# martinruenz/maskfusion

Measured on NVIDIA H100. Metric: frames/sec on 640x480 .klg replay, higher is better.
Workload: dtype f32

## Files before the change

### maskfusion_b200/csrc/mf_surfel.cu

```cuda
#include "mf_common.cuh"
#include "mf_kernels.h"
#include "mf_host.h"

namespace mfb {

#define MAX_POINT_SIZE 2047.0f

__global__ void __launch_bounds__(256) k_index_project(const float4* __restrict__ pos, const float4* __restrict__ col,
                                                       const uint32_t* __restrict__ countPtr, const DevPose* __restrict__ dpose, Cam cam, int W, int H,
                                                       float maxDepth, float ftime, float ftimeDelta,
                                                       unsigned long long* __restrict__ key)
{
    const Rt tinv = dpose->tinv;
    const uint32_t count = *countPtr;
    for (uint32_t id = blockIdx.x * blockDim.x + threadIdx.x; id < count; id += gridDim.x * blockDim.x) {
        float4 p = ldStream(pos + id);
        float lastTime = ldStream(col + id).w;
        float3 ph = xform(tinv, make_float3(p.x, p.y, p.z));
        if (ph.z > maxDepth || ph.z <= 0 || ftime - lastTime > ftimeDelta) continue;
        float x = ((cam.fx * ph.x) / ph.z) + cam.cx;
        float y = ((cam.fy * ph.y) / ph.z) + cam.cy;
        float zn = ph.z / maxDepth;
        if (!(zn < 1.0f)) continue;
        float fx_ = floorf(x), fy_ = floorf(y);
// ... 307 lines not shown
        for (uint32_t i = lane; i < staged; i += 32) cand[gbase + i] = sBuf[warp][i];
        __syncwarp();
        staged = 0;
    };
    const uint32_t stride = gridDim.x * blockDim.x;
    float4 vpN = make_float4(0, 0, 0, 0), vcN = vpN;
    { const uint32_t e0 = blockIdx.x * blockDim.x + threadIdx.x; if (e0 < count) { vpN = pos[e0]; vcN = col[e0]; } }
    for (uint32_t base = blockIdx.x * blockDim.x; base < total; base += stride) {
        const uint32_t e = base + threadIdx.x;
        bool valid = false, need = false, noWindow = false;
        const bool isOld = e < count;
        float4 vp = vpN, vc = vcN;
        if (e + stride < count) { vpN = pos[e + stride]; vcN = col[e + stride]; }
        if (isOld) valid = true;
        else if (e < total) { uint32_t p = e - count; if (aflag[p] == 2) { vp = m0[p]; vc = m1[p]; valid = true; } }
        if (valid) {
            float3 lp = xform(P.tinv, make_float3(vp.x, vp.y, vp.z));
            float x = ((P.cam.fx * lp.x) / lp.z) + P.cam.cx;
            float y = ((P.cam.fy * lp.y) / lp.z) + P.cam.cy;
            need = ftime - vc.w < P.ftimeDelta && lp.z > 0 && x > 0 && y > 0 && x < cols && y < rows;
            if (indexKey && isOld && !(lp.z > indexMaxDepth || lp.z <= 0 || ftime - vc.w > P.ftimeDelta)) {
                const float zn = lp.z / indexMaxDepth;
                const float fx_ = floorf(x), fy_ = floorf(y);
                if (zn < 1.0f && fx_ >= 0 && fy_ >= 0 && fx_ < cols && fy_ < rows) {
                    const unsigned long long k = ((unsigned long long)__float_as_uint(zn) << 32) | e;
                    unsigned long long* dst = indexKey + ((int)fy_ * P.W + (int)fx_);
                    if (k < *dst) atomicMin(dst, k);
                    if (!need) { need = true; noWindow = true; }
                }
            }
            if (!need) {
                const float w0 = vp.w, t0 = vc.w;
                bool k = cleanFinish(vp, vc, x, y, lp.z, 0, 0, P, depthFilt, mask);
                if (isOld) { if (vp.w != w0) pos[e].w = vp.w; if (vc.w != t0) col[e].w = vc.w; }
                else { uint32_t p = e - count; m0[p].w = vp.w; m1[p].w = vc.w; }
                keep[e] = k ? 1 : 0;
            }
        } else if (e < total) keep[e] = 0;
        const unsigned nb = __ballot_sync(0xffffffffu, need);
        if (nb) {
            if (staged + 32 > CAND_BUF / 8) flush();
            if (need) sBuf[warp][staged + __popc(nb & ((1u << lane) - 1))] = noWindow ? (e | 0x80000000u) : e;
            staged += (uint32_t)__popc(nb);
            __syncwarp();
        }
    }
    if (staged) flush();
}

template <bool PACKED>
__global__ void __launch_bounds__(256, 4) k_clean_p2(float4* __restrict__ pos, float4* __restrict__ col, const float4* __restrict__ nrm,
                                                  const uint32_t* __restrict__ countPtr, float4* __restrict__ m0, float4* __restrict__ m1,
                                                  const float4* __restrict__ m2, CleanParams P, const DevPose* __restrict__ dpose, CleanTexels cleanTex,
                                                  const float* __restrict__ depthFilt, const uint8_t* __restrict__ mask, uint8_t* __restrict__ keep,
                                                  const uint32_t* __restrict__ cand, const uint32_t* __restrict__ candCount)
{
    P.tinv = dpose->tinv;
    const uint32_t count = *countPtr, n = *candCount;
    const float cols = (float)P.W, rows = (float)P.H;
    for (uint32_t j = blockIdx.x * blockDim.x + threadIdx.x; j < n; j += gridDim.x * blockDim.x) {
        const uint32_t ce_ = cand[j];
        const bool noWindow = (ce_ >> 31) != 0;
        const uint32_t e = ce_ & 0x7fffffffu;
        const bool isOld = e < count;
        const uint32_t p = e - count;
        float4 vp, vc, vn;
        if (isOld) { vp = pos[e]; vc = col[e]; vn = nrm[e]; } else { vp = m0[p]; vc = m1[p]; vn = m2[p]; }
        const float w0 = vp.w, t0 = vc.w;
        float3 lp = xform(P.tinv, make_float3(vp.x, vp.y, vp.z));
        float x = ((P.cam.fx * lp.x) / lp.z) + P.cam.cx;
        float y = ((P.cam.fy * lp.y) / lp.z) + P.cam.cy;
        float3 ln = normalize3(rotate(P.tinv, make_float3(vn.x, vn.y, vn.z)));
        CleanEntry ce; ce.xn = x / cols; ce.yn = y / rows; ce.lx = lp.x; ce.ly = lp.y; ce.lz = lp.z; ce.init = vc.z; ce.rad = vn.w; ce.lnz = fabsf(ln.z);
        int c1 = 0, c2 = 0;
        if (!noWindow) cleanWindow<PACKED>(ce, P, cleanTex, c1, c2);
        bool k = cleanFinish(vp, vc, x, y, lp.z, c1, c2, P, depthFilt, mask);
        if (isOld) { if (vp.w != w0) pos[e].w = vp.w; if (vc.w != t0) col[e].w = vc.w; }
        else { m0[p].w = vp.w; m1[p].w = vc.w; }
        keep[e] = k ? 1 : 0;
    }
}

__global__ void __launch_bounds__(256) k_keep_block_sums(const uint8_t* __restrict__ keep, const uint32_t* __restrict__ countPtr, int Ppix,
                                                         uint32_t* __restrict__ blockSums, uint32_t* __restrict__ candCount, uint32_t* __restrict__ ticket)
{
    const uint32_t total = *countPtr + (uint32_t)Ppix;
    const uint32_t nblk = (total + SCAN_BLOCK - 1) / SCAN_BLOCK;
    if (blockIdx.x == 0 && threadIdx.x == 0) { *candCount = 0; *ticket = 0; }
    const uint32_t lane = threadIdx.x & 31, gw = (blockIdx.x * blockDim.x + threadIdx.x) >> 5, nw = (gridDim.x * blockDim.x) >> 5;
    for (uint32_t blk = gw; blk < nblk; blk += nw) {
        const uint32_t e0 = blk * SCAN_BLOCK + lane * 16;
        uint4 v = make_uint4(0, 0, 0, 0);
        if (e0 < total) v = *reinterpret_cast<const uint4*>(keep + e0);
        if (e0 < total && total - e0 < 16) {
            const uint32_t r = total - e0;
            uint32_t w[4] = {v.x, v.y, v.z, v.w};
#pragma unroll
            for (int q = 0; q < 4; ++q) { const uint32_t lo = (uint32_t)q * 4; w[q] = r <= lo ? 0u : (r - lo >= 4 ? w[q] : (w[q] & ((1u << (8 * (r - lo))) - 1u))); }
            v = make_uint4(w[0], w[1], w[2], w[3]);
        }
        uint32_t c = __popc(v.x & 0x01010101u) + __popc(v.y & 0x01010101u) + __popc(v.z & 0x01010101u) + __popc(v.w & 0x01010101u);
#pragma unroll
        for (int off = 16; off > 0; off >>= 1) c += __shfl_xor_sync(0xffffffffu, c, off);
        if (lane == 0) blockSums[blk] = c;
    }
}

__global__ void __launch_bounds__(1024) k_scan_block_sums(uint32_t* __restrict__ blockSums, const uint32_t* __restrict__ countPtr,
                                                          int extra, uint32_t capacity, uint32_t* __restrict__ newCount, uint32_t* __restrict__ firstMoved)
{
    const uint32_t total = *countPtr + (uint32_t)extra;
    const uint32_t nblk = (total + SCAN_BLOCK - 1) / SCAN_BLOCK;
    __shared__ uint32_t wtot[32];
    __shared__ uint32_t sFirst;
    if (threadIdx.x == 0) sFirst = nblk;
    __syncthreads();
    const uint32_t per = (nblk + 1023) / 1024;
    const uint32_t b0 = threadIdx.x * per, b1 = min(b0 + per, nblk);
    uint32_t run = 0, first = 0xffffffffu;
    for (uint32_t i = b0; i < b1; ++i) { const uint32_t v = blockSums[i]; run += v; if (v != SCAN_BLOCK && first == 0xffffffffu) first = i; }
    if (first != 0xffffffffu) atomicMin(&sFirst, first);
    const int lane = threadIdx.x & 31, warp = threadIdx.x >> 5;
    uint32_t incl = run;
#pragma unroll
    for (int off = 1; off < 32; off <<= 1) { const uint32_t t = __shfl_up_sync(0xffffffffu, incl, off); if (lane >= off) incl += t; }
    if (lane == 31) wtot[warp] = incl;
    __syncthreads();
    if (warp == 0) {
        uint32_t w = wtot[lane], wi = w;
#pragma unroll
        for (int off = 1; off < 32; off <<= 1) { const uint32_t t = __shfl_up_sync(0xffffffffu, wi, off); if (lane >= off) wi += t; }
        wtot[lane] = wi - w;
        if (lane == 31) { *newCount = wi < capacity ? wi : capacity; }
    }
    __syncthreads();
    uint32_t offs = wtot[warp] + incl - run;
    for (uint32_t i = b0; i < b1; ++i) { const uint32_t v = blockSums[i]; blockSums[i] = offs; offs += v; }
    if (threadIdx.x == 0) { firstMoved[0] = sFirst; firstMoved[1] = nblk; }
}

__global__ void __launch_bounds__(SCAN_BLOCK) k_clean_scatter(const float4* __restrict__ pos, const float4* __restrict__ col, const float4* __restrict__ nrm,
                                                              const uint32_t* __restrict__ countPtr, const float4* __restrict__ m0,
                                                              const float4* __restrict__ m1, const float4* __restrict__ m2, int Ppix,
                                                              const uint8_t* __restrict__ keep, const uint32_t* __restrict__ blockOffs,
                                                              uint32_t capacity, float4* __restrict__ opos, float4* __restrict__ ocol,
                                                              float4* __restrict__ onrm)
{
    const uint32_t count = *countPtr;
    const uint32_t total = count + (uint32_t)Ppix;
    const uint32_t nblk = (total + SCAN_BLOCK - 1) / SCAN_BLOCK;
    __shared__ uint32_t wsum[SCAN_BLOCK / 32];
    for (uint32_t blk = blockIdx.x; blk < nblk; blk += gridDim.x) {
        uint32_t e = blk * SCAN_BLOCK + threadIdx.x;
        bool k = e < total && keep[e];
        unsigned bal = __ballot_sync(0xffffffffu, k);
        int lane = threadIdx.x & 31, warp = threadIdx.x >> 5;
        if (lane == 0) wsum[warp] = __popc(bal);
        __syncthreads();
        uint32_t woff = 0;
        for (int w = 0; w < warp; ++w) woff += wsum[w];
        uint32_t dst = blockOffs[blk] + woff + __popc(bal & ((1u << lane) - 1));
        if (k && dst < capacity) {
            float4 a, b, c;
            if (e < count) { a = ldStream(pos + e); b = ldStream(col + e); c = ldStream(nrm + e); }
            else { uint32_t p = e - count; a = m0[p]; b = m1[p]; c = m2[p]; }
            stStream(opos + dst, a); stStream(ocol + dst, b); stStream(onrm + dst, c);
        }
        __syncthreads();
    }
}

__global__ void __launch_bounds__(SCAN_BLOCK) k_clean_compact(float4* __restrict__ pos, float4* __restrict__ col, float4* __restrict__ nrm,
                                                              const uint32_t* __restrict__ countPtr, const float4* __restrict__ m0,
                                                              const float4* __restrict__ m1, const float4* __restrict__ m2, int Ppix,
                                                              const uint8_t* __restrict__ keep, const uint32_t* __restrict__ blockOffs,
                                                              uint32_t capacity, uint32_t* __restrict__ ticket, uint32_t* __restrict__ loaded,
                                                              const uint32_t* __restrict__ firstMoved, uint32_t epoch)
{
    const uint32_t count = *countPtr;
    const uint32_t total = count + (uint32_t)Ppix;
    const uint32_t nblk = (total + SCAN_BLOCK - 1) / SCAN_BLOCK;
    const uint32_t first = *firstMoved;
    __shared__ uint32_t wsum[SCAN_BLOCK / 32];
    __shared__ uint32_t sBlk[2];
    const int lane = threadIdx.x & 31, warp = threadIdx.x >> 5;
    if (threadIdx.x == 0) sBlk[0] = first + atomicAdd(ticket, 1u);
    __syncthreads();
    for (uint32_t it = 0;; ++it) {
        const uint32_t blk = sBlk[it & 1];
        if (blk >= nblk) break;
        if (threadIdx.x == 0) sBlk[(it + 1) & 1] = first + atomicAdd(ticket, 1u);
        const uint32_t e = blk * SCAN_BLOCK + threadIdx.x;
        const bool k = e < total && keep[e];
        const unsigned bal = __ballot_sync(0xffffffffu, k);
        if (lane == 0) wsum[warp] = __popc(bal);
        __syncthreads();
        uint32_t woff = 0, nb = 0;
#pragma unroll
        for (int w = 0; w < SCAN_BLOCK / 32; ++w) { const uint32_t c = wsum[w]; if (w < warp) woff += c; nb += c; }
        const uint32_t off = blockOffs[blk];
        const uint32_t dst = off + woff + __popc(bal & ((1u << lane) - 1));
        const bool isOld = e < count;
        const bool move = k && dst < capacity && !(isOld && dst == e);
        float4 a = make_float4(0, 0, 0, 0), b = a, c = a;
        if (move) {
            if (isOld) { a = __ldcg(pos + e); b = __ldcg(col + e); c = __ldcg(nrm + e); }
            else { const uint32_t p = e - count; a = m0[p]; b = m1[p]; c = m2[p]; }
        }
        const unsigned probe = __float_as_uint(a.x) & __float_as_uint(b.y) & __float_as_uint(c.z);
        __syncthreads_or(probe == 0x7fedcba9u);
        if (threadIdx.x == 0) {
            asm volatile("st.release.gpu.global.u32 [%0], %1;" ::"l"(loaded + blk), "r"(epoch) : "memory");
            if (nb) {
                const uint32_t s0 = off / SCAN_BLOCK, s1 = (off + nb - 1) / SCAN_BLOCK;
                for (uint32_t s = s0; s <= s1 && s < blk; ++s) {
                    if (s < first) continue;
                    unsigned v;
                    do { asm volatile("ld.acquire.gpu.global.u32 %0, [%1];" : "=r"(v) : "l"(loaded + s) : "memory"); } while (v != epoch);
                }
            }
        }
        __syncthreads();
        if (move) { stStream(pos + dst, a); stStream(col + dst, b); stStream(nrm + dst, c); }
    }
}

struct SplatVS { float3 pos; float conf; float3 n; float rad, size, xw, yw; bool ok; };

MF_D SplatVS splatVertex(float4 p, float4 c, float4 nr, const Rt& tinv, Cam cam, int W, int H, float maxDepth,
                         float confThreshold, float ftime, float fmaxTime, float ftimeDelta)
{
    SplatVS o; o.ok = false;
    float3 ph = xform(tinv, make_float3(p.x, p.y, p.z));
    if (ph.z > maxDepth || ph.z < 0 || p.w < confThreshold || ftime - c.w > ftimeDelta || c.w > fmaxTime) return o;
    o.pos = ph; o.conf = p.w;
    o.n = normalize3(rotate(tinv, make_float3(nr.x, nr.y, nr.z)));
    o.rad = nr.w;
    float3 x1 = normalize3(make_float3(o.n.y - o.n.z, -o.n.x, o.n.x));
    x1 = make_float3(x1.x * o.rad * 1.41421356f, x1.y * o.rad * 1.41421356f, x1.z * o.rad * 1.41421356f);
    float3 y1 = cross3(o.n, x1);
    float px[4], py[4];
#pragma unroll
    for (int q = 0; q < 4; ++q) {
        float3 d = (q == 0 || q == 3) ? x1 : y1;
        float sg = (q < 2) ? 1.0f : -1.0f;
        float3 pp = make_float3(ph.x + sg * d.x, ph.y + sg * d.y, ph.z + sg * d.z);
        px[q] = ((cam.fx * pp.x) / pp.z) + cam.cx;
        py[q] = ((cam.fy * pp.y) / pp.z) + cam.cy;
    }
    float xmin = fminf(px[0], fminf(px[1], fminf(px[2], px[3]))), xmax = fmaxf(px[0], fmaxf(px[1], fmaxf(px[2], px[3])));
    float ymin = fminf(py[0], fminf(py[1], fminf(py[2], py[3]))), ymax = fmaxf(py[0], fmaxf(py[1], fmaxf(py[2], py[3])));
    float sz = fmaxf(0.0f, fmaxf(fabsf(xmax - xmin), fabsf(ymax - ymin)));
    if (!(sz >= 1.0f)) sz = 1.0f;
    if (sz > MAX_POINT_SIZE) sz = MAX_POINT_SIZE;
    o.size = sz;
    o.xw = ((cam.fx * ph.x) / ph.z) + cam.cx;
    o.yw = ((cam.fy * ph.y) / ph.z) + cam.cy;
    if (!(o.xw >= 0 && o.xw <= (float)W && o.yw >= 0 && o.yw <= (float)H)) return o;
    if (!(ph.z / maxDepth <= 1.0f)) return o;
    o.ok = true;
    return o;
}

MF_D float3 pixelRay(Cam cam, float fcx, float fcy)
{
    return normalize3(make_float3((fcx - cam.cx) / cam.fx, (fcy - cam.cy) / cam.fy, 1.0f));
}
__global__ void k_ray_table(Cam cam, int W, int H, float4* __restrict__ tab)
{
    int px = blockIdx.x * blockDim.x + threadIdx.x, py = blockIdx.y * blockDim.y + threadIdx.y;
    if (px >= W || py >= H) return;
    float3 l = pixelRay(cam, (float)px + 0.5f, (float)py + 0.5f);
    tab[py * W + px] = make_float4(l.x, l.y, l.z, 0.f);
}

MF_D bool splatFragmentRay(const SplatVS& v, float3 l, float3& cp)
{
    float t = dot3(v.pos, v.n) / dot3(l, v.n);
    cp = make_float3(t * l.x, t * l.y, t * l.z);
    float sqrRad = v.rad * v.rad;
    float3 d = sub3(cp, v.pos);
    return !(dot3(d, d) > sqrRad);
}
MF_D bool splatFragment(const SplatVS& v, Cam cam, float fcx, float fcy, float3& cp) { return splatFragmentRay(v, pixelRay(cam, fcx, fcy), cp); }

MF_D void splatRange(const SplatVS& v, int W, int H, int& x0, int& x1, int& y0, int& y1)
{
    float h = v.size * 0.5f;
    float lo = ceilf(v.xw - h - 0.5f), hi = ceilf(v.xw + h - 0.5f) - 1.0f;
    x0 = lo < 0 ? 0 : (int)lo; x1 = hi > (float)(W - 1) ? W - 1 : (int)hi;
    lo = ceilf(v.yw - h - 0.5f); hi = ceilf(v.yw + h - 0.5f) - 1.0f;
    y0 = lo < 0 ? 0 : (int)lo; y1 = hi > (float)(H - 1) ? H - 1 : (int)hi;
}

#define SPLAT_SEG 8
#ifndef SPLAT_BS
#define SPLAT_BS 128
#endif
#ifndef SPLAT_MIN_BLOCKS
#define SPLAT_MIN_BLOCKS 8
#endif
#define SPLAT_Q 64

struct __align__(16) SplatEntry { float px, py, pz, pn, nx, ny, nz, rad; int x0, y0, w; uint32_t id; };

MF_D void splatExact(const SplatEntry& e, int pix, const float4* __restrict__ rayTab, unsigned long long* __restrict__ key, float maxDepth)
{
    SplatVS sv; sv.pos = make_float3(e.px, e.py, e.pz); sv.n = make_float3(e.nx, e.ny, e.nz); sv.rad = e.rad;
    const float4 l4 = __ldg(rayTab + pix);
    float3 cp;
    if (!splatFragmentRay(sv, make_float3(l4.x, l4.y, l4.z), cp)) return;
    const float fd = (cp.z / (2 * maxDepth)) + 0.5f;
    if (!(fd >= 0.0f && fd < 1.0f)) return;
    const unsigned long long k = ((unsigned long long)__float_as_uint(fd) << 32) | e.id;
    if (k < key[pix]) atomicMin(key + pix, k);
}

__global__ void __launch_bounds__(SPLAT_BS, SPLAT_MIN_BLOCKS) k_splat_project(const float4* __restrict__ pos, const float4* __restrict__ col, const float4* __restrict__ nrm,
                                                       const uint32_t* __restrict__ countPtr, const DevPose* __restrict__ dpose, Cam cam, int W, int H,
                                                       float maxDepth, float confThreshold, float ftime, float fmaxTime, float ftimeDelta,
                                                       uint32_t drawBase, const float4* __restrict__ rayTab, unsigned long long* __restrict__ key)
{
    constexpr int NW = SPLAT_BS / 32;
    static_assert(SPLAT_BS % 32 == 0 && SPLAT_BS <= 256, "the queue packs the entry slot into 8 bits");
    __shared__ SplatEntry ent[2][SPLAT_BS];
    __shared__ int offs[2][SPLAT_BS];
    __shared__ __align__(16) float4 spos[SPLAT_BS];
    __shared__ uint32_t queue[NW][SPLAT_Q];
    __shared__ int wtot[NW], wcnt[NW];
    __shared__ Rt tinv;
    __shared__ float inv2md;
    __shared__ __align__(8) unsigned long long bar;
    const uint32_t count = *countPtr;
    const int lane = threadIdx.x & 31, warp = threadIdx.x >> 5;
    const uint32_t stride = gridDim.x * SPLAT_BS;
    const unsigned barAddr = (unsigned)__cvta_generic_to_shared(&bar);
    const unsigned sposAddr = (unsigned)__cvta_generic_to_shared(spos);
    auto fetch = [&](uint32_t b) {
        const unsigned bytes = min((uint32_t)SPLAT_BS, count - b) * 16u;
        asm volatile("mbarrier.arrive.expect_tx.shared::cta.b64 _, [%0], %1;" ::"r"(barAddr), "r"(bytes) : "memory");
        asm volatile("cp.async.bulk.shared::cluster.global.mbarrier::complete_tx::bytes [%0], [%1], %2, [%3];"
                     ::"r"(sposAddr), "l"(pos + b), "r"(bytes), "r"(barAddr) : "memory");
    };
    if (threadIdx.x < 12) tinv.m[threadIdx.x] = dpose->tinv.m[threadIdx.x];
    if (threadIdx.x == 0) {
        inv2md = 1.0f / (2 * maxDepth);
        asm volatile("mbarrier.init.shared::cta.b64 [%0], 1;" ::"r"(barAddr));
        asm volatile("fence.mbarrier_init.release.cluster;" ::: "memory");
        if (blockIdx.x * SPLAT_BS < count) fetch(blockIdx.x * SPLAT_BS);
    }
    __syncthreads();
    unsigned parity = 0;
    for (uint32_t base = blockIdx.x * SPLAT_BS; base < count; base += stride, parity ^= 1u) {
        const uint32_t id = base + threadIdx.x;
        SplatVS v; v.ok = false;
        int x0 = 0, x1 = -1, y0 = 0, y1 = -1;
        asm volatile(
            "{\n\t.reg .pred p;\n\t"
            "SPLAT_WAIT:\n\t"
            "mbarrier.try_wait.parity.shared::cta.b64 p, [%0], %1;\n\t"
            "@!p bra SPLAT_WAIT;\n\t}" ::"r"(barAddr), "r"(parity) : "memory");
        if (id < count) {
            const float4 p = spos[threadIdx.x];
            float3 ph = xform(tinv, make_float3(p.x, p.y, p.z));
            const float cxw = ((cam.fx * ph.x) / ph.z) + cam.cx, cyw = ((cam.fy * ph.y) / ph.z) + cam.cy;
            if (!(ph.z > maxDepth || ph.z < 0 || p.w < confThreshold) && cxw >= 0 && cxw <= (float)W && cyw >= 0 && cyw <= (float)H) {
                float4 c = ldStream(col + id), nr = ldStream(nrm + id);
                v = splatVertex(p, c, nr, tinv, cam, W, H, maxDepth, confThreshold, ftime, fmaxTime, ftimeDelta);
                if (v.ok) splatRange(v, W, H, x0, x1, y0, y1);
            }
        }
        const bool draw = v.ok && x1 >= x0 && y1 >= y0;
        const int nunit = draw ? (y1 - y0 + 1) * ((x1 - x0 + SPLAT_SEG) / SPLAT_SEG) : 0;
        int incl = nunit;
#pragma unroll
        for (int o = 1; o < 32; o <<= 1) { int t = __shfl_up_sync(0xffffffffu, incl, o); if (lane >= o) incl += t; }
        unsigned db = __ballot_sync(0xffffffffu, draw);
        if (lane == 31) wtot[warp] = incl;
        if (lane == 0) wcnt[warp] = __popc(db);
        __syncthreads();
        if (threadIdx.x == 0 && base + stride < count) {
            asm volatile("fence.proxy.async.shared::cta;" ::: "memory");
            fetch(base + stride);
        }
        SplatEntry* __restrict__ E = ent[parity];
        int* __restrict__ O = offs[parity];
        int fbase = 0, sbase = 0, total = 0, nent = 0;
#pragma unroll
        for (int w = 0; w < NW; ++w) { if (w < warp) { fbase += wtot[w]; sbase += wcnt[w]; } total += wtot[w]; nent += wcnt[w]; }
        if (draw) {
            const int slot = sbase + __popc(db & ((1u << lane) - 1));
            SplatEntry e; e.px = v.pos.x; e.py = v.pos.y; e.pz = v.pos.z; e.pn = dot3(v.pos, v.n); e.nx = v.n.x; e.ny = v.n.y; e.nz = v.n.z; e.rad = v.rad;
            e.x0 = x0; e.y0 = y0; e.w = x1 - x0 + 1; e.id = drawBase + id;
            E[slot] = e;
            O[slot] = fbase + incl - nunit;
        }
        __syncthreads();
        uint32_t* __restrict__ q = queue[warp];
        int qn = 0;
        for (int ub = threadIdx.x - lane + blockIdx.y * SPLAT_BS; ub < total; ub += SPLAT_BS * gridDim.y) {
            const int u = ub + lane;
            int slot = 0, pix = 0, n = 0;
            if (u < total) {
                int lo = 0, hi = nent - 1;
                while (lo < hi) { int mid = (lo + hi + 1) >> 1; if (O[mid] <= u) lo = mid; else hi = mid - 1; }
                slot = lo;
                const int t = u - O[slot], w = E[slot].w, x0e = E[slot].x0;
                const int nseg = (w + SPLAT_SEG - 1) / SPLAT_SEG;
                const int row = t / nseg, xs = x0e + (t - row * nseg) * SPLAT_SEG;
                n = min(SPLAT_SEG, x0e + w - xs);
                pix = (E[slot].y0 + row) * W + xs;
            }
            const int nmax = __reduce_max_sync(0xffffffffu, n);
            for (int i = 0; i < nmax; ++i, ++pix) {
                bool cand = false;
                if (i < n) {
                    const float4 pp = *reinterpret_cast<const float4*>(&E[slot].px), nr = *reinterpret_cast<const float4*>(&E[slot].nx);
                    const float4 l4 = __ldg(rayTab + pix);
                    const unsigned long long cur = key[pix];
                    const float ta = __fdividef(pp.w, dot3(make_float3(l4.x, l4.y, l4.z), make_float3(nr.x, nr.y, nr.z)));
                    cand = cur == KEY_EMPTY || !(__fmaf_rn(ta * l4.z, inv2md, 0.5f) > __uint_as_float((unsigned)(cur >> 32)) * 1.00001f);
                    if (cand) {
                        const float ax = __fmaf_rn(ta, l4.x, -pp.x), ay = __fmaf_rn(ta, l4.y, -pp.y), az = __fmaf_rn(ta, l4.z, -pp.z);
                        const float re = nr.w + 8e-6f * fabsf(ta);
                        cand = !(__fmaf_rn(ax, ax, __fmaf_rn(ay, ay, az * az)) > re * re * 1.0001f);
                    }
                }
                const unsigned m = __ballot_sync(0xffffffffu, cand);
                if (cand) q[qn + __popc(m & ((1u << lane) - 1))] = (uint32_t)pix << 8 | (uint32_t)slot;
                qn += __popc(m);
                if (qn >= 32) {
                    qn -= 32;
                    __syncwarp();
                    const uint32_t it = q[qn + lane];
                    __syncwarp();
                    splatExact(E[it & 255u], (int)(it >> 8), rayTab, key, maxDepth);
                }
            }
        }
        __syncwarp();
        if (lane < qn) {
            const uint32_t it = q[lane];
            splatExact(E[it & 255u], (int)(it >> 8), rayTab, key, maxDepth);
        }
    }
}

__global__ void k_splat_resolve(const float4* __restrict__ pos, const float4* __restrict__ col, const float4* __restrict__ nrm,
                                const DevPose* __restrict__ dpose, Cam cam, int W, int H, float maxDepth, float confThreshold, float ftime, float fmaxTime,
                                float ftimeDelta, const float4* __restrict__ rayTab, unsigned long long* __restrict__ key,
                                uchar4* __restrict__ image, float4* __restrict__ vertexConf, float4* __restrict__ normalRad,
                                uint16_t* __restrict__ timeTex,
                                int doFill, const float* __restrict__ depthFilt, const uchar4* __restrict__ rgb, int ptVN, int ptImg,
                                uchar4* __restrict__ fillImage, float4* __restrict__ fillVertex, float4* __restrict__ fillNormal,
                                uint32_t* __restrict__ nonBlackSamples)
{
    const Rt tinv = dpose->tinv;
    int px = blockIdx.x * blockDim.x + threadIdx.x, py = blockIdx.y * blockDim.y + threadIdx.y;
    if (px >= W || py >= H) return;
    int i = py * W + px;
    unsigned long long k = key[i];
    uchar4 im = make_uchar4(0, 0, 0, 0);
    float4 vc = make_float4(0, 0, 0, 0), nr = vc;
    uint16_t tt = 0;
    if (k != KEY_EMPTY) {
        key[i] = KEY_EMPTY;
        uint32_t id = (uint32_t)(k & 0xffffffffull);
        float4 p = pos[id], c = col[id], n = nrm[id];
        SplatVS v = splatVertex(p, c, n, tinv, cam, W, H, maxDepth, confThreshold, ftime, fmaxTime, ftimeDelta);
        float3 cp; float fcx = (float)px + 0.5f, fcy = (float)py + 0.5f;
        const float4 l4 = __ldg(rayTab + i);
        splatFragmentRay(v, make_float3(l4.x, l4.y, l4.z), cp);
        float3 cl = decodeColor(c.x);
        im = make_uchar4((uint8_t)(int)floorf(cl.x * 255.0f + 0.5f), (uint8_t)(int)floorf(cl.y * 255.0f + 0.5f),
                         (uint8_t)(int)floorf(cl.z * 255.0f + 0.5f), 255);
        float z = cp.z;
        vc = make_float4((fcx - cam.cx) * z * (1.f / cam.fx), (fcy - cam.cy) * z * (1.f / cam.fy), z, v.conf);
        nr = make_float4(v.n.x, v.n.y, v.n.z, v.rad);
        tt = (uint16_t)(uint32_t)c.z;
    }
    image[i] = im; vertexConf[i] = vc; normalRad[i] = nr; timeTex[i] = tt;
    if (nonBlackSamples && (px % 20) == 10 && (py % 20) == 10 && px / 20 < W / 20 && py / 20 < H / 20) {
        if (im.x > 0 && im.y > 0 && im.z > 0) atomicAdd(nonBlackSamples, 1u);
    }
    if (doFill) {
        const float ifx = 1.0f / cam.fx, ify = 1.0f / cam.fy;
        float3 vp = getVertex(depthFilt, W, H, px, py, (float)px, (float)py, cam, ifx, ify);
        fillVertex[i] = (vc.z == 0 || ptVN) ? make_float4(vp.x, vp.y, vp.z, 1.f) : vc;
        if (nr.z == 0 || ptVN) {
            float3 n = normalForward(depthFilt, W, H, px, py, cam, ifx, ify, vp);
            fillNormal[i] = make_float4(n.x, n.y, n.z, 1.f);
        } else fillNormal[i] = nr;
        float sum = ((float)im.x / 255.0f + (float)im.y / 255.0f) + (float)im.z / 255.0f;
        fillImage[i] = (sum == 0 || ptImg) ? rgb[i] : im;
    }
}

__global__ void __launch_bounds__(SCAN_BLOCK) k_init_flags(const float* __restrict__ depthRaw, const float* __restrict__ depthFilt,
                                                           int W, int H, float maxDepth, uint8_t* __restrict__ fr, uint8_t* __restrict__ ff,
                                                           uint32_t* __restrict__ sumR, uint32_t* __restrict__ sumF)
{
    const int P = W * H;
    __shared__ uint32_t ws[2][SCAN_BLOCK / 32];
    int p = blockIdx.x * SCAN_BLOCK + threadIdx.x;
    bool kr = false, kf = false;
    if (p < P) {
        int i = p / H, j = p - i * H;
        float zr = depthRaw[j * W + i], zf = depthFilt[j * W + i];
        kr = !(zr <= 0 || zr > maxDepth);
        kf = !(zf <= 0 || zf > maxDepth);
        fr[p] = kr; ff[p] = kf;
    }
    unsigned br = __ballot_sync(0xffffffffu, kr), bf = __ballot_sync(0xffffffffu, kf);
    if ((threadIdx.x & 31) == 0) { ws[0][threadIdx.x >> 5] = __popc(br); ws[1][threadIdx.x >> 5] = __popc(bf); }
    __syncthreads();
    if (threadIdx.x == 0) {
        uint32_t a = 0, b = 0;
        for (int w = 0; w < SCAN_BLOCK / 32; ++w) { a += ws[0][w]; b += ws[1][w]; }
        sumR[blockIdx.x] = a; sumF[blockIdx.x] = b;
    }
}

__global__ void __launch_bounds__(SCAN_BLOCK) k_init_scatter(const uchar4* __restrict__ rgb, const float* __restrict__ depthRaw,
                                                             const float* __restrict__ depthFilt, Cam cam, int W, int H, int time,
                                                             const uint8_t* __restrict__ fr, const uint8_t* __restrict__ ff,
                                                             const uint32_t* __restrict__ offR, const uint32_t* __restrict__ offF,
                                                             uint32_t capacity, float4* __restrict__ pos, float4* __restrict__ col,
                                                             float4* __restrict__ nrm)
{
    const int P = W * H;
    __shared__ uint32_t ws[2][SCAN_BLOCK / 32];
    int p = blockIdx.x * SCAN_BLOCK + threadIdx.x;
    bool kr = p < P && fr[p], kf = p < P && ff[p];
    unsigned br = __ballot_sync(0xffffffffu, kr), bf = __ballot_sync(0xffffffffu, kf);
    int lane = threadIdx.x & 31, warp = threadIdx.x >> 5;
    if (lane == 0) { ws[0][warp] = __popc(br); ws[1][warp] = __popc(bf); }
    __syncthreads();
    uint32_t wr = 0, wf = 0;
    for (int w = 0; w < warp; ++w) { wr += ws[0][w]; wf += ws[1][w]; }
    if (p >= P) return;
    int i = p / H, j = p - i * H;
    const float ifx = 1.0f / cam.fx, ify = 1.0f / cam.fy;
    float tcx = (float)(((double)((float)i / (float)W)) + 1.0 / (double)(2 * (float)W));
    float tcy = (float)(((double)((float)j / (float)H)) + 1.0 / (double)(2 * (float)H));
    float x = tcx * (float)W, y = tcy * (float)H;
    if (kr) {
        uint32_t dst = offR[blockIdx.x] + wr + __popc(br & ((1u << lane) - 1));
        if (dst < capacity) {
            float3 vp = getVertex(depthRaw, W, H, i, j, x, y, cam, ifx, ify);
            uchar4 c8 = rgb[j * W + i];
            pos[dst] = make_float4(vp.x, vp.y, vp.z, surfelConfidence(x, y, 1.0f, cam.cx, cam.cy));
            col[dst] = make_float4(encodeColor((float)c8.x / 255.0f, (float)c8.y / 255.0f, (float)c8.z / 255.0f), 0.f, 1.f, (float)time);
        }
    }
    if (kf) {
        uint32_t dst = offF[blockIdx.x] + wf + __popc(bf & ((1u << lane) - 1));
        if (dst < capacity) {
            float3 vp = getVertex(depthFilt, W, H, i, j, x, y, cam, ifx, ify);
            float3 nl = normalCentral(depthFilt, W, H, i, j, x, y, cam, ifx, ify, vp);
            nrm[dst] = make_float4(nl.x, nl.y, nl.z, surfelRadius(vp.z, nl.z, ifx, ify));
        }
    }
}

__global__ void __launch_bounds__(1024) k_scan_small(uint32_t* __restrict__ a, int n, uint32_t capacity, uint32_t* __restrict__ total)
{
    __shared__ uint32_t sh[1024];
    __shared__ uint32_t carry;
    if (threadIdx.x == 0) carry = 0;
    __syncthreads();
    for (int base = 0; base < n; base += 1024) {
        int i = base + threadIdx.x;
        uint32_t v = i < n ? a[i] : 0;
        sh[threadIdx.x] = v;
        __syncthreads();
        for (int off = 1; off < 1024; off <<= 1) {
            uint32_t t = threadIdx.x >= off ? sh[threadIdx.x - off] : 0;
            __syncthreads();
            sh[threadIdx.x] += t;
            __syncthreads();
        }
        uint32_t incl = sh[threadIdx.x];
        if (i < n) a[i] = carry + incl - v;
        __syncthreads();
        if (threadIdx.x == 1023) carry += incl;
        __syncthreads();
    }
    if (threadIdx.x == 0 && total) *total = carry < capacity ? carry : capacity;
}

__global__ void k_fill_u32(uint32_t* p, uint32_t v, size_t n)
{
    size_t i = (size_t)blockIdx.x * blockDim.x + threadIdx.x;
    if (i < n) p[i] = v;
}
__global__ void k_fill_u64(unsigned long long* p, unsigned long long v, size_t n)
{
    size_t i = (size_t)blockIdx.x * blockDim.x + threadIdx.x;
    if (i < n) p[i] = v;
}
__global__ void k_zero_f4(float4* p, uint32_t from, uint32_t to)
{
    uint32_t i = from + blockIdx.x * blockDim.x + threadIdx.x;
    if (i < to) p[i] = make_float4(0, 0, 0, 0);
}

__global__ void k_planes_to_aos(const float4* __restrict__ pos, const float4* __restrict__ col, const float4* __restrict__ nrm, uint32_t n, float4* __restrict__ out)
{
    uint32_t i = blockIdx.x * blockDim.x + threadIdx.x;
    if (i >= n) return;
    out[(size_t)i * 3] = pos[i]; out[(size_t)i * 3 + 1] = col[i]; out[(size_t)i * 3 + 2] = nrm[i];
}
__global__ void k_aos_to_planes(const float4* __restrict__ in, uint32_t n, float4* __restrict__ pos, float4* __restrict__ col, float4* __restrict__ nrm)
{
    uint32_t i = blockIdx.x * blockDim.x + threadIdx.x;
    if (i >= n) return;
    pos[i] = in[(size_t)i * 3]; col[i] = in[(size_t)i * 3 + 1]; nrm[i] = in[(size_t)i * 3 + 2];
}

static int g_numSMs = 0;
void set_num_sms(int n) { g_numSMs = n > 0 ? n : 132; }
int num_sms()
{
    if (!g_numSMs) { int dev = 0, n = 0; cudaGetDevice(&dev); cudaDeviceGetAttribute(&n, cudaDevAttrMultiProcessorCount, dev); set_num_sms(n); }
    return g_numSMs;
}
static inline int persistentBlocks(int perSM) { return num_sms() * perSM; }

struct Pose2 { float p[16], l[16]; };
__global__ void k_set_pose(DevPose* d, Pose2 in)
{
    if (threadIdx.x == 0 && blockIdx.x == 0) derivePose(d, in.p, in.l);
}
void launch_set_pose(DevPose* d, const float* pose16, const float* lastPose16, Enq q)
{
    Pose2 in;
    for (int k = 0; k < 16; ++k) { in.p[k] = pose16[k]; in.l[k] = lastPose16[k]; }
    launch(q, nullptr, k_set_pose, 1, 32, 0, d, in);
}

void launch_fill_u32(uint32_t* p, uint32_t v, size_t n, Enq q) { if (n) launch(q, nullptr, k_fill_u32, (unsigned)((n + 255) / 256), 256, 0, p, v, n); }
void launch_fill_u64(uint64_t* p, uint64_t v, size_t n, Enq q) { if (n) launch(q, nullptr, k_fill_u64, (unsigned)((n + 255) / 256), 256, 0, (unsigned long long*)p, v, n); }

void launch_predict_indices(const SurfelPlanes& sp, const uint32_t* count, const DevPose* tinv, Cam cam, int W, int H, float maxDepth, int time,
                            int timeDelta, uint64_t* key, uint32_t* idx, float4* vertConf, float4* colorTime, float4* normRad, float4* cleanTex, float cleanConf, Enq q)
{
    launch(q, "k_index_project", k_index_project, persistentBlocks(8), 256, 0, sp.pos, sp.col, count, tinv, cam, W, H, maxDepth, (float)time, (float)timeDelta,
           (unsigned long long*)key);
    int P = W * H;
    launch(q, "k_index_resolve", k_index_resolve, (P + 255) / 256, 256, 0, sp.pos, sp.col, sp.nrm, tinv, P, (unsigned long long*)key, idx, vertConf, colorTime, normRad, cleanTex, cleanConf, (float)time);
}

void launch_associate(const uchar4* rgb, const float* depthRaw, const float* depthFilt, const uint8_t* mask, const uint32_t* idx,
                      const float4* vertConf, const float4* normRad, const DevPose* pose, Cam cam, int W, int H, float maxDepth, int time,
                      float weighting, uint8_t maskID, uint8_t* flag, uint32_t* best, float4* const* meas, uint32_t* slot, Enq q)
{
    dim3 b(32, 8), g((W + 31) / 32, (H + 7) / 8);
    launch(q, "k_associate", k_associate, g, b, 0, rgb, depthRaw, depthFilt, mask, idx, vertConf, normRad, pose, cam, W, H, maxDepth, time, weighting, maskID,
           flag, best, meas[0], meas[1], meas[2], slot);
}

void launch_fuse_update(const uint8_t* flag, const uint32_t* best, float4* const* meas, uint32_t* slot, int P, int time,
                        const SurfelPlanes& sp, Enq q)
{
    launch(q, "k_fuse_update", k_fuse_update, (P + 255) / 256, 256, 0, flag, best, meas[0], meas[1], meas[2], slot, P, time, sp.pos, sp.col, sp.nrm);
    launch(q, "k_slot_release", k_slot_release, (P + 255) / 256, 256, 0, flag, best, P, slot);
}

void launch_clean(const SurfelPlanes& src, const SurfelPlanes& dst, const uint32_t* count, uint32_t* newCount, uint32_t capacity,
                  const uint8_t* aflag, float4* const* meas, const DevPose* tinv, Cam cam, int W, int H, int time, int timeDelta, float confThreshold,
                  float outlierCoeff, uint8_t maskID, const CleanWindowImages& win,
                  const float* depthFilt, const uint8_t* mask, uint8_t* keep, uint32_t* blockSums, uint32_t* cand, uint32_t* candCount, Enq q,
                  const CleanInPlace& inplace, const IndexFused* fused)
{
    const CleanTexels texels{win.packed, win.vertConf, win.colorTime, win.idx};
    CleanParams P;
    P.tinv = Rt{};
    P.cam = cam; P.W = W; P.H = H; P.time = time; P.ftimeDelta = (float)timeDelta; P.confThreshold = confThreshold;
    P.outlierCoeff = outlierCoeff; P.maskID = maskID;
    int Ppix = W * H;
    int blocks = persistentBlocks(4);
    launch(q, "k_clean_p1", k_clean_p1, persistentBlocks(8), 256, 0, src.pos, src.col, count, aflag, meas[0], meas[1], Ppix, P, tinv, depthFilt, mask, keep, cand, candCount,
           fused ? (unsigned long long*)fused->key : nullptr, fused ? fused->maxDepth : 0.f);
    if (fused) {
        launch(q, "k_index_resolve", k_index_resolve, (Ppix + 255) / 256, 256, 0, src.pos, src.col, src.nrm, tinv, Ppix, (unsigned long long*)fused->key, fused->idx,
               fused->vertConf, fused->colorTime, fused->normRad, fused->cleanTex, confThreshold, (float)time);
    }
    launch(q, "k_clean_p2", texels.packed ? k_clean_p2<true> : k_clean_p2<false>, persistentBlocks(8), 256, 0, src.pos, src.col, src.nrm, count, meas[0], meas[1], meas[2],
           P, tinv, texels, depthFilt, mask, keep, cand, candCount);
    launch(q, "k_keep_block_sums", k_keep_block_sums, persistentBlocks(8), 256, 0, keep, count, Ppix, blockSums, candCount, inplace.ticket);
    launch(q, "k_scan_block_sums", k_scan_block_sums, 1, 1024, 0, blockSums, count, Ppix, capacity, newCount, inplace.firstMoved);
    if (!inplace.pingPong) {
        launch(q, "k_clean_compact", k_clean_compact, blocks, SCAN_BLOCK, 0, src.pos, src.col, src.nrm, count, meas[0], meas[1], meas[2], Ppix, keep, blockSums, capacity,
               inplace.ticket, inplace.loaded, inplace.firstMoved, inplace.epoch);
    } else {
        launch(q, "k_clean_scatter", k_clean_scatter, blocks, SCAN_BLOCK, 0, src.pos, src.col, src.nrm, count, meas[0], meas[1], meas[2], Ppix, keep, blockSums, capacity,
               dst.pos, dst.col, dst.nrm);
    }
}

void launch_ray_table(Cam cam, int W, int H, float4* tab, Enq q)
{
    dim3 b(32, 8), g((W + 31) / 32, (H + 7) / 8);
    launch(q, nullptr, k_ray_table, g, b, 0, cam, W, H, tab);
}

static dim3 splatGrid(uint32_t capacity, int W, int H)
{
    if ((size_t)W * H > (1u << 24)) throw CudaError{"splat rasteriser: more than 2^24 pixels (its exact-path queue keeps 24-bit pixel indices)"};
    static const int perSM = [] {
        int n = 0;
        cudaCheck(cudaOccupancyMaxActiveBlocksPerMultiprocessor(&n, k_splat_project, SPLAT_BS, 0), "k_splat_project occupancy");
        if (n < 1) throw CudaError{"k_splat_project does not fit on an SM"};
        return n;
    }();
    const int persistent = persistentBlocks(perSM);
    if (capacity == 0 || capacity >= (1u << 20)) return dim3(persistent);
    const int cols = (int)std::min<uint32_t>((capacity + SPLAT_BS - 1) / SPLAT_BS, (uint32_t)persistent);
    return dim3(cols, 8);
}
void launch_combined_predict(const SurfelPlanes& sp, const uint32_t* count, const DevPose* tinv, Cam cam, int W, int H, float maxDepth,
                             float confThreshold, int time, int maxTime, int timeDelta, const float4* rayTab, uint64_t* key, uchar4* image, float4* vertexConf,
                             float4* normalRad, uint16_t* timeTex, int doFill, const float* depthFilt, const uchar4* rgb, int ptVN, int ptImg,
                             uchar4* fillImage, float4* fillVertex, float4* fillNormal, uint32_t* nonBlackSamples, Enq q, uint32_t capacity)
{
    launch(q, "k_splat_project", k_splat_project, splatGrid(capacity, W, H), SPLAT_BS, 0, sp.pos, sp.col, sp.nrm, count, tinv, cam, W, H, maxDepth, confThreshold, (float)time,
           (float)maxTime, (float)timeDelta, 0u, rayTab, (unsigned long long*)key);
    if (nonBlackSamples) cudaMemsetAsync(nonBlackSamples, 0, sizeof(uint32_t), q.s);
    dim3 b(32, 8), g((W + 31) / 32, (H + 7) / 8);
// ... 31 lines not shown
```

Baseline: 758.3.

## Rewrite splat prefilter with analytic rays and incremental approximate reciprocal

The per-pixel conservative prefilter in the splat kernel no longer loads the ray table or the full 64-bit key. It computes the ray analytically from the inverse focal lengths, hoists per-segment normal and plane terms out of the pixel loop, and advances the ray x-coordinate incrementally. The divide becomes an approximate reciprocal and only the high 32-bit depth half of the key is read. Error-bound constants plus a near-grazing fallback (|den| < sg) keep the filter conservative before the exact pass, at the risk of subtle misclassification if the bounds are wrong.

```diff
diff --git a/maskfusion_b200/csrc/mf_surfel.cu b/maskfusion_b200/csrc/mf_surfel.cu
--- a/maskfusion_b200/csrc/mf_surfel.cu
+++ b/maskfusion_b200/csrc/mf_surfel.cu
@@ -633,6 +633,18 @@
 #endif
 #define SPLAT_Q 64
 
+#define SPLAT_GMAX 8.0f
+constexpr float SPLAT_DEPTH_BASE = 0.5f - 136.0f * 0x1p-24f;
+constexpr float SPLAT_DISC_Z = 280.0f * 0x1p-24f;
+constexpr float SPLAT_DISC_R = 1.0f + 16.0f * 0x1p-24f;
+
+MF_D float rcpApprox(float x)
+{
+    float r;
+    asm("rcp.approx.ftz.f32 %0, %1;" : "=f"(r) : "f"(x));
+    return r;
+}
+
 struct __align__(16) SplatEntry { float px, py, pz, pn, nx, ny, nz, rad; int x0, y0, w; uint32_t id; };
 
 MF_D void splatExact(const SplatEntry& e, int pix, const float4* __restrict__ rayTab, unsigned long long* __restrict__ key, float maxDepth)
@@ -660,8 +672,9 @@
     __shared__ uint32_t queue[NW][SPLAT_Q];
     __shared__ int wtot[NW], wcnt[NW];
     __shared__ Rt tinv;
-    __shared__ float inv2md;
+    __shared__ float inv2md, ifx, ify;
     __shared__ __align__(8) unsigned long long bar;
+    const unsigned* keyHi = reinterpret_cast<const unsigned*>(key) + 1;
     const uint32_t count = *countPtr;
     const int lane = threadIdx.x & 31, warp = threadIdx.x >> 5;
     const uint32_t stride = gridDim.x * SPLAT_BS;
@@ -676,6 +689,7 @@
     if (threadIdx.x < 12) tinv.m[threadIdx.x] = dpose->tinv.m[threadIdx.x];
     if (threadIdx.x == 0) {
         inv2md = 1.0f / (2 * maxDepth);
+        ifx = 1.0f / cam.fx; ify = 1.0f / cam.fy;
         asm volatile("mbarrier.init.shared::cta.b64 [%0], 1;" ::"r"(barAddr));
         asm volatile("fence.mbarrier_init.release.cluster;" ::: "memory");
         if (blockIdx.x * SPLAT_BS < count) fetch(blockIdx.x * SPLAT_BS);
@@ -729,9 +743,11 @@
         __syncthreads();
         uint32_t* __restrict__ q = queue[warp];
         int qn = 0;
+        const float i2m = inv2md, dx = ifx, dy = ify;
         for (int ub = threadIdx.x - lane + blockIdx.y * SPLAT_BS; ub < total; ub += SPLAT_BS * gridDim.y) {
             const int u = ub + lane;
             int slot = 0, pix = 0, n = 0;
+            float nx = 0.f, px = 0.f, py = 0.f, pz = 0.f, rw = 0.f, ru = 0.f, rv = 0.f, a = 0.f, sg = 0.f, cz = 0.f;
             if (u < total) {
                 int lo = 0, hi = nent - 1;
                 while (lo < hi) { int mid = (lo + hi + 1) >> 1; if (O[mid] <= u) lo = mid; else hi = mid - 1; }
@@ -741,21 +757,29 @@
                 const int row = t / nseg, xs = x0e + (t - row * nseg) * SPLAT_SEG;
                 n = min(SPLAT_SEG, x0e + w - xs);
                 pix = (E[slot].y0 + row) * W + xs;
+                const float4 pp = *reinterpret_cast<const float4*>(&E[slot].px), nr = *reinterpret_cast<const float4*>(&E[slot].nx);
+                ru = __fmul_rn(__fsub_rn((float)xs + 0.5f, cam.cx), dx);
+                rv = __fmul_rn(__fsub_rn((float)(E[slot].y0 + row) + 0.5f, cam.cy), dy);
+                const float ubound = __fmaf_rn(8.0f, dx, fabsf(ru));
+                const float ipn = rcpApprox(pp.w);
+                a = __fmul_rn(__fmaf_rn(rv, nr.y, nr.z), ipn);
+                nx = __fmul_rn(nr.x, ipn);
+                sg = __fmul_rn(__fmaf_rn(ubound, fabsf(nr.x), __fmaf_rn(fabsf(rv), fabsf(nr.y), fabsf(nr.z))), fabsf(ipn) * (1.0f / SPLAT_GMAX));
+                cz = __fmul_rn(__fmaf_rn(0.5f, __fmaf_rn(ubound, ubound, __fmul_rn(rv, rv)), 1.0f), SPLAT_DISC_Z);
+                rw = __fmul_rn(nr.w, SPLAT_DISC_R);
+                px = pp.x; py = pp.y; pz = pp.z;
             }
             const int nmax = __reduce_max_sync(0xffffffffu, n);
-            for (int i = 0; i < nmax; ++i, ++pix) {
+            for (int i = 0; i < nmax; ++i, ++pix, ru = __fadd_rn(ru, dx)) {
                 bool cand = false;
                 if (i < n) {
-                    const float4 pp = *reinterpret_cast<const float4*>(&E[slot].px), nr = *reinterpret_cast<const float4*>(&E[slot].nx);
-                    const float4 l4 = __ldg(rayTab + pix);
-                    const unsigned long long cur = key[pix];
-                    const float ta = __fdividef(pp.w, dot3(make_float3(l4.x, l4.y, l4.z), make_float3(nr.x, nr.y, nr.z)));
-                    cand = cur == KEY_EMPTY || !(__fmaf_rn(ta * l4.z, inv2md, 0.5f) > __uint_as_float((unsigned)(cur >> 32)) * 1.00001f);
-                    if (cand) {
-                        const float ax = __fmaf_rn(ta, l4.x, -pp.x), ay = __fmaf_rn(ta, l4.y, -pp.y), az = __fmaf_rn(ta, l4.z, -pp.z);
-                        const float re = nr.w + 8e-6f * fabsf(ta);
-                        cand = !(__fmaf_rn(ax, ax, __fmaf_rn(ay, ay, az * az)) > re * re * 1.0001f);
-                    }
+                    const float den = __fmaf_rn(ru, nx, a);
+                    const float z = rcpApprox(den);
+                    const float cur = __uint_as_float(keyHi[2 * pix]);
+                    const float ax = __fmaf_rn(z, ru, -px), ay = __fmaf_rn(z, rv, -py), az = __fsub_rn(z, pz);
+                    const float re = __fmaf_rn(fabsf(z), cz, rw);
+                    const bool drop = __fmaf_rn(z, i2m, SPLAT_DEPTH_BASE) > cur || __fmaf_rn(ax, ax, __fmaf_rn(ay, ay, __fmul_rn(az, az))) > __fmul_rn(re, re);
+                    cand = fabsf(den) < sg || !drop;
                 }
                 const unsigned m = __ballot_sync(0xffffffffu, cand);
                 if (cand) q[qn + __popc(m & ((1u << lane) - 1))] = (uint32_t)pix << 8 | (uint32_t)slot;
```

Measured after the change: 758.3, median of 6. No clear change (+0.0%).
